# Lqm26/BMCNet-ESR

Measured on AMD Instinct MI355X. Metric: LR-voxel-frames/sec x4 SR train step, NFS-shaped 180x240 (BASELINE configs[1] / [2]), f32, higher is better.
Workload: dtype f32; 1 GPU; BMCNet(scale=4, n_c=128, n_b=5) x4 SR train step, NFS-shaped 180x240 (BASELINE configs[1] / [2]) -> 720x960, bs=4/GPU, arithmetic fp32 (native fp32 MFMA; 3x3 convolutions through Winograd F(4x4,3x3) / F(2x2,3x3) transforms in fp32), SEQL=9 SEQN=2 (8 windows BPTT), event scatter + fwd + MSE + bwd + Adam(amsgrad); global_batch=4, parallelism=dp1, rccl_ranks=1, rccl_initialised_before_headline_run=False

## Files before the change

### bmcnet-esr_amd/csrc/wino4_wgrad.hip

```cpp
#include "bmc_common.h"
#include "dma_ring.h"

namespace {

struct Wgrad4K {
    SrcDev a;
    SrcDev x;
    int B, H, W;
    int TY, SX;
    int nstages, nsplit;
    float* part;
    float* bias_part;
};

typedef float f32x2 __attribute__((ext_vector_type(2)));

__device__ __forceinline__ const float* uni(const float* p) {
    const unsigned long long v = reinterpret_cast<unsigned long long>(p);
    const unsigned lo = __builtin_amdgcn_readfirstlane((unsigned)v), hi = __builtin_amdgcn_readfirstlane((unsigned)(v >> 32));
    return reinterpret_cast<const float*>(((unsigned long long)hi << 32) | lo);
}

constexpr int NPW = 18;
constexpr int TS = 4;
constexpr int CH = 64;
constexpr int PIMG = TS * CH;
constexpr int IMG = NPW * PIMG;
constexpr int SIMG = 2 * IMG;
constexpr int XPC = 23, YPC = 16;
constexpr int RAWX = XPC * 256;
constexpr int RAWF = (XPC + YPC) * 256;
constexpr int NPC = XPC + YPC;
constexpr int PPW = 5;
constexpr int LDSF = 2 * RAWF + 2 * SIMG;
static_assert(LDSF * 4 <= 160 * 1024, "LDS budget");

constexpr int dma_gap(const int j) { return 2 * j; }
constexpr int TR_READ = 0, TR_COMB = 3, TR_OUT = 10;

template <int I, int N>
struct W4gFor {
    template <class F>
    static __device__ __forceinline__ void run(F&& f) {
        f(std::integral_constant<int, I>{});
        W4gFor<I + 1, N>::run(f);
    }
};
template <int N>
struct W4gFor<N, N> {
    template <class F>
    static __device__ __forceinline__ void run(F&&) {}
};

template <int TG, int ROLE>
__device__ __forceinline__ void wgrad4_body(const Wgrad4K& a, float* const lds, const int split, const int chh, const int kh) {
    const int tid = threadIdx.x, lane = tid & 63;
    const int wave = __builtin_amdgcn_readfirstlane(tid >> 6);
    float* const rawb = lds;
    float* const imgb = lds + 2 * RAWF;
    const unsigned lds_raw = lds_addr(rawb);

    const int pg = wave >> 2, cb = (wave >> 1) & 1, kb = wave & 1;
    const int l31 = lane & 31, lh = lane >> 5;
    const int aoff = 3 * pg * PIMG + lh * CH + 32 * cb + l31;
    const int boff = IMG + 3 * pg * PIMG + lh * CH + 32 * kb + l31;
    f32x16 acc[9];
#pragma unroll
    for (int i = 0; i < 9; ++i)
#pragma unroll
        for (int r = 0; r < 16; ++r) acc[i][r] = 0.f;

    unsigned poff[PPW];
    unsigned pof[PPW];
    unsigned pla[PPW];
    unsigned pxm = 0;
    auto piece_of = [&](const int j) { return min(wave + 8 * j, NPC - 1); };
    const bool has_last = wave + 8 * (PPW - 1) < NPC;
    auto slot_of = [&](const int p, int& r, int& c) __attribute__((always_inline)) {
        if (p < XPC) { const int q = 4 * p + (lane >> 4); r = q / 18; c = q - 18 * r; return q < 90; }
        const int q = 4 * (p - XPC) + (lane >> 4); r = q >> 4; c = q & 15;
        return true;
    };
#pragma unroll
    for (int j = 0; j < PPW; ++j) {
        const int p = piece_of(j);
        int r, c;
        const bool real = slot_of(p, r, c);
        poff[j] = real ? (unsigned)(((r * a.W + c) * 128 + (lane & 15) * 4) * 4) : 0u;
        pof[j] = poff[j];
        pla[j] = lds_raw + (unsigned)(p * 1024);
        pxm |= p < XPC ? 1u << j : 0u;
    }
    unsigned zm = 0;
    static_assert(PPW <= 32, "zm is a bit mask");

    const int per_img = a.TY * a.SX;
    const int st0 = (int)((long long)a.nstages * split / a.nsplit), st1 = (int)((long long)a.nstages * (split + 1) / a.nsplit);
    int nb = st0 / per_img, nty, nsx;
    {
        const int r = st0 - nb * per_img;
        nty = r / a.SX; nsx = r - nty * a.SX;
    }
    nb = __builtin_amdgcn_readfirstlane(nb); nty = __builtin_amdgcn_readfirstlane(nty); nsx = __builtin_amdgcn_readfirstlane(nsx);
    const float* xbat = nullptr;
    const float* ybat = nullptr;
    const float* xrow = nullptr;
    const float* yrow = nullptr;
    bool rowborder = false;
    auto row_setup = [&]() __attribute__((always_inline)) {
        xbat = uni(src_batch_ptr(a.x, nb) + kh * CH);
        ybat = uni(src_batch_ptr(a.a, nb) + chh * CH);
        const int y0 = 4 * nty - 1 + TG;
        rowborder = y0 < 0 || y0 + 4 >= a.H;
        xrow = xbat + (long long)y0 * a.W * 128;
        yrow = ybat + (long long)(4 * nty) * a.W * 128;
    };
    row_setup();

    const float* rq_xs = nullptr;
    const float* rq_ys = nullptr;
    unsigned rq_lo = 0;
    auto rq_begin = [&](const int rb) __attribute__((always_inline)) {
        rq_lo = (unsigned)(rb * RAWF * 4);
        const int y0 = 4 * nty - 1 + TG, x0 = 16 * nsx - 1;
        const bool border = rowborder || nsx == 0 || x0 + 17 >= a.W;
        rq_xs = border ? xbat : xrow + x0 * 128;
        rq_ys = border ? ybat : yrow + (x0 + 1) * 128;
        zm = 0;
        if (border) {
            asm volatile("; image border" ::: "memory");
#pragma unroll
            for (int j = 0; j < PPW; ++j) {
                const bool isx = (pxm >> j) & 1;
                int r, c;
                const bool real = slot_of(piece_of(j), r, c);
                const int y = (isx ? y0 : y0 + 1 - TG) + r, x = (isx ? x0 : x0 + 1) + c;
                const bool inside = y >= 0 && y < a.H && x >= 0 && x < a.W;
                const int yc = min(max(y, 0), a.H - 1), xc = min(max(x, 0), a.W - 1);
                pof[j] = real ? (unsigned)(((yc * a.W + xc) * 128 + (lane & 15) * 4) * 4) : 0u;
                zm |= (real && !inside) ? (1u << j) : 0u;
            }
        } else {
#pragma unroll
            for (int j = 0; j < PPW; ++j) pof[j] = poff[j];
        }
        if (!has_last) zm &= ~(1u << (PPW - 1));
        if (++nsx == a.SX) {
            nsx = 0;
            if (++nty == a.TY) { nty = 0; ++nb; }
            row_setup();
        }
    };
    auto rq_piece = [&](const int j) __attribute__((always_inline)) {
        if (j == PPW - 1 && !has_last) return;
        dma16_sgpr<1>(((pxm >> j) & 1) ? rq_xs : rq_ys, pof[j], pla[j] + rq_lo);
    };
    auto patch = [&](const int rb) __attribute__((always_inline)) {
        if (__builtin_amdgcn_ballot_w64(zm != 0) == 0) return;
#pragma unroll
        for (int j = 0; j < PPW; ++j)
            if ((zm >> j) & 1) *reinterpret_cast<f32x4*>(rawb + (pla[j] - lds_raw) / 4 + rb * RAWF + lane * 4) = f32x4{0.f, 0.f, 0.f, 0.f};
    };

    const int pt = 2 * (wave >> 2) + (lane >> 5), cp = lane & 31;
    constexpr int NK = ROLE == 0 ? 3 : 4;
    constexpr int NC = ROLE == 3 ? 4 : 6;
    constexpr int KS = ROLE == 0 ? 2 * 18 * CH : (ROLE == 3 ? 16 * CH : 18 * CH);
    const int tsrc = (ROLE == 0 ? 4 * pt * CH : (ROLE == 3 ? RAWX + 4 * pt * CH : ((1 - TG) * 18 + 4 * pt) * CH)) + 2 * cp;
    const int tdst = (ROLE == 3 ? 0 : IMG + (ROLE == 0 ? (TG == 0 ? 0 : 2) : (TG == 0 ? 1 : 0) + (ROLE == 2 ? 1 : 0)) * 6 * PIMG) + pt * CH + 2 * cp;
    f32x2 td[NC][NK];
    f32x2 tw[3][NC];
    f32x2 bsum = {0.f, 0.f};
    auto ld2 = [](const float* p) __attribute__((always_inline)) { return *reinterpret_cast<const f32x2*>(p); };
    auto st2 = [](float* p, const f32x2 v) __attribute__((always_inline)) { *reinterpret_cast<f32x2*>(p) = v; };
    auto tgap = [&](auto gc, const float* const raw, float* const img) __attribute__((always_inline)) {
        constexpr int G = decltype(gc)::value;
        constexpr int cr = G - TR_READ, cc = G - TR_COMB;
        if constexpr (cr >= 0 && cr < NC) {
#pragma unroll
            for (int k = 0; k < NK; ++k) td[cr][k] = ld2(raw + tsrc + k * KS + cr * CH);
        }
        if constexpr (cc >= 0 && cc < NC) {
            const f32x2* const d = td[cc];
            if constexpr (ROLE == 0) {
                tw[0][cc] = 4.f * d[0] - 5.f * d[1] + d[2];
            } else if constexpr (ROLE < 3) {
                constexpr float al = TG == 0 ? -4.f : -1.f;
                constexpr float ga = (TG == 0 ? 1.f : 2.f) * (ROLE == 2 ? -1.f : 1.f);
                tw[0][cc] = (d[3] + al * d[1]) + ga * (d[2] + al * d[0]);
            } else {
                constexpr float ka = TG == 0 ? 1.f : 4.f, la = TG == 0 ? 1.f : 2.f;
                const f32x2 p = d[0] + ka * d[2], q = d[1] + ka * d[3];
                if (TG == 0) { tw[0][cc] = d[0]; tw[1][cc] = p + la * q; tw[2][cc] = p - la * q; }
                else { tw[0][cc] = p + la * q; tw[1][cc] = p - la * q; tw[2][cc] = d[3]; }
            }
        }
        constexpr int ko = G - TR_OUT;
        if constexpr (ko >= 0 && ko < 6 && (ko & 1) == 0) {
            constexpr int k = ko >> 1;
            if constexpr (ROLE < 3) {
                const f32x2* const w = tw[0];
                float* const dst = img + tdst;
                if (k == 0) {
                    st2(dst, 4.f * w[0] - 5.f * w[2] + w[4]);
                    st2(dst + 5 * PIMG, 4.f * w[1] - 5.f * w[3] + w[5]);
                } else if (k == 1) {
                    const f32x2 ta = w[4] - 4.f * w[2], tb = w[3] - 4.f * w[1];
                    st2(dst + PIMG, ta + tb);
                    st2(dst + 2 * PIMG, ta - tb);
                } else {
                    const f32x2 tc = w[4] - w[2], te = w[3] - w[1];
                    st2(dst + 3 * PIMG, tc + 2.f * te);
                    st2(dst + 4 * PIMG, tc - 2.f * te);
                }
            } else {
                const f32x2* const w = tw[k];
                float* const dst = img + tdst + 6 * k * PIMG;
                const f32x2 s = w[0] + w[2], t = w[1] + w[3], p = w[0] + 4.f * w[2], q = w[1] + 4.f * w[3];
                const f32x2 m1 = s + t;
                st2(dst, w[0]);
                st2(dst + PIMG, m1);
                st2(dst + 2 * PIMG, s - t);
                st2(dst + 3 * PIMG, p + 2.f * q);
                st2(dst + 4 * PIMG, p - 2.f * q);
                st2(dst + 5 * PIMG, w[3]);
                if (TG == 0 && k == 1) bsum += m1;
            }
        }
    };

    auto stage = [&](const int it, auto reqc, auto morec) __attribute__((always_inline)) {
        constexpr bool REQ = decltype(reqc)::value, MORE = decltype(morec)::value;
        const float* const img = imgb + (it & 1) * SIMG;
        const float* const traw = rawb + ((it + 1) & 1) * RAWF;
        float* const timg = imgb + ((it + 1) & 1) * SIMG;
        if (REQ) rq_begin(it & 1);
        float af[3][2], bf[3][2];
        auto frag = [&](const int i) __attribute__((always_inline)) {
            const int u = i / 3, j = i - 3 * u, sl = i % 3;
#pragma unroll
            for (int ks = 0; ks < 2; ++ks) {
                af[sl][ks] = img[aoff + (6 * u + j) * PIMG + 2 * ks * CH];
                bf[sl][ks] = img[boff + (6 * u + j) * PIMG + 2 * ks * CH];
            }
        };
        __builtin_amdgcn_sched_barrier(0);
        frag(0);
        frag(1);
        W4gFor<0, 9>::run([&](auto ic) __attribute__((always_inline)) {
            constexpr int i = decltype(ic)::value;
            __builtin_amdgcn_sched_barrier(0);
            if (i + 2 < 9) frag(i + 2);
            __builtin_amdgcn_sched_barrier(0);
            W4gFor<0, 2>::run([&](auto kc) __attribute__((always_inline)) {
                constexpr int ks = decltype(kc)::value, g = 2 * i + ks;
                acc[i] = __builtin_amdgcn_mfma_f32_32x32x2f32(af[i % 3][ks], bf[i % 3][ks], acc[i], 0, 0, 0);
                if (REQ) {
#pragma unroll
                    for (int j = 0; j < PPW; ++j)
                        if (dma_gap(j) == g) rq_piece(j);
                }
                if (MORE) tgap(std::integral_constant<int, g>{}, traw, timg);
                __builtin_amdgcn_sched_barrier(0);
            });
        });
        dma_wait<0>();
        if (REQ) patch(it & 1);
        ring_publish();
    };

    const int n = st1 - st0;
    if (n <= 0) return;
    rq_begin(0);
#pragma unroll
    for (int j = 0; j < PPW; ++j) rq_piece(j);
    dma_wait<0>();
    patch(0);
    ring_publish();
    if (n > 1) {
        rq_begin(1);
#pragma unroll
        for (int j = 0; j < PPW; ++j) rq_piece(j);
    }
    W4gFor<0, 18>::run([&](auto gc) __attribute__((always_inline)) { tgap(gc, rawb, imgb); });
    dma_wait<0>();
    if (n > 1) patch(1);
    ring_publish();
    using T_ = std::true_type;
    using F_ = std::false_type;
    int it = 0;
    for (; it + 2 < n; ++it) stage(it, T_{}, T_{});
    if (it + 1 < n) stage(it++, F_{}, T_{});
    stage(it, F_{}, F_{});

    {
        float* const P = a.part + ((((long long)split * 8 + (TG * 4 + chh * 2 + kh)) * 8 + wave) * 9) * 1024 + lane * 4;
#pragma unroll
        for (int i = 0; i < 9; ++i)
#pragma unroll
            for (int m = 0; m < 4; ++m)
                stg16(P + (i * 4 + m) * 256, f32x4{acc[i][4 * m], acc[i][4 * m + 1], acc[i][4 * m + 2], acc[i][4 * m + 3]});
    }
    if (TG == 0 && kh == 0 && a.bias_part) {
        if (ROLE == 3) *reinterpret_cast<f32x2*>(lds + pt * CH + 2 * cp) = bsum;
        __syncthreads();
        if (tid < CH) a.bias_part[(long long)split * 128 + 64 * chh + tid] = (lds[tid] + lds[CH + tid]) + (lds[2 * CH + tid] + lds[3 * CH + tid]);
    }
}

template <int TG>
__device__ __forceinline__ void wgrad4_role(const Wgrad4K& a, float* const lds, const int split, const int chh, const int kh) {
    switch (__builtin_amdgcn_readfirstlane(threadIdx.x >> 6) & 3) {
        case 0: wgrad4_body<TG, 0>(a, lds, split, chh, kh); break;
        case 1: wgrad4_body<TG, 1>(a, lds, split, chh, kh); break;
        case 2: wgrad4_body<TG, 2>(a, lds, split, chh, kh); break;
        default: wgrad4_body<TG, 3>(a, lds, split, chh, kh); break;
    }
}

__global__ __launch_bounds__(512, 2) void wino4_wgrad_kernel(const Wgrad4K a) {
    __shared__ __attribute__((aligned(16))) float lds[LDSF];
    int type, split;
    if ((a.nsplit & 7) == 0) {
        const int j = blockIdx.x >> 3;
        type = j & 7; split = (j >> 3) * 8 + (blockIdx.x & 7);
    } else {
        type = blockIdx.x & 7; split = blockIdx.x >> 3;
    }
    const int chh = (type >> 1) & 1, kh = type & 1;
    if (type & 4) wgrad4_role<1>(a, lds, split, chh, kh);
    else wgrad4_role<0>(a, lds, split, chh, kh);
}

constexpr int RED_THREADS = 288, RED_GROUPS = 512;
__global__ __launch_bounds__(RED_THREADS) void wino4_wgrad_reduce_kernel(const float* __restrict__ part, int nsplit, float* __restrict__ dw,
                                                                        int ldw, int k0, int accumulate, const float* __restrict__ bias_part,
                                                                        float* __restrict__ db) {
    constexpr long long SSTRIDE = 36ll * 16384;
    const int t = threadIdx.x;
    if ((int)blockIdx.x == RED_GROUPS) {
        if (t >= 128) return;
        float s = 0.f;
        int i = 0;
        for (; i + 8 <= nsplit; i += 8) {
            float q[8];
#pragma unroll
            for (int k = 0; k < 8; ++k) q[k] = bias_part[(long long)(i + k) * 128 + t];
#pragma unroll
            for (int k = 0; k < 8; ++k) s += q[k];
        }
        for (; i < nsplit; ++i) s += bias_part[(long long)i * 128 + t];
        db[t] = accumulate ? db[t] + s : s;
        return;
    }
    __shared__ f32x4 U[36][8];
    const int c = blockIdx.x >> 5, r = blockIdx.x & 31;
    const int chh = c >> 3, kh = (c >> 2) & 1, cb = (c >> 1) & 1, kb = c & 1;
    const int m = r >> 3, lane0 = 8 * (r & 7);
    {
        const int p = t >> 3, qi = t & 7;
        const int xi = p / 6, nu = p - 6 * xi;
        const int type = (xi / 3) * 4 + chh * 2 + kh, wv = (nu / 3) * 4 + cb * 2 + kb, a9 = 3 * (xi % 3) + nu % 3;
        const float* const ps = part + (((long long)type * 8 + wv) * 9 + a9) * 1024 + m * 256 + (lane0 + qi) * 4;
        f32x4 u = {0.f, 0.f, 0.f, 0.f};
        int s = 0;
        for (; s + 8 <= nsplit; s += 8) {
            f32x4 q[8];
#pragma unroll
            for (int k = 0; k < 8; ++k) q[k] = ldg16(ps + (s + k) * SSTRIDE);
#pragma unroll
            for (int k = 0; k < 8; ++k) u += q[k];
        }
        for (; s < nsplit; ++s) u += ldg16(ps + s * SSTRIDE);
        U[p][qi] = u;
    }
    __syncthreads();
    const float G[6][3] = {{0.25f, 0.f, 0.f}, {-1.f / 6, -1.f / 6, -1.f / 6}, {-1.f / 6, 1.f / 6, -1.f / 6},
                           {1.f / 24, 1.f / 12, 1.f / 6}, {1.f / 24, -1.f / 12, 1.f / 6}, {0.f, 0.f, 1.f}};
    const int e = t / 72, r2 = t - 72 * e, qi = r2 / 9, tap = r2 - 9 * qi, ti = tap / 3, tj = tap - 3 * ti;
    float o = 0.f;
#pragma unroll
    for (int k = 0; k < 8; ++k) {
        float tk = 0.f;
#pragma unroll
        for (int p = k; p < 36; p += 8) {
            const int xi = p / 6, nu = p - 6 * xi;
            float gi = 0.f, gj = 0.f;
#pragma unroll
            for (int q = 0; q < 3; ++q) { gi = q == ti ? G[xi][q] : gi; gj = q == tj ? G[nu][q] : gj; }
            tk += (gi * gj) * U[p][qi][e];
        }
        o += tk;
    }
    const int co = 64 * chh + 32 * cb + 8 * m + 4 * (lane0 >> 5) + e, ci = 64 * kh + 32 * kb + (lane0 & 31) + qi;
    float* const d = dw + ((long long)co * ldw + k0 + ci) * 9 + tap;
    *d = accumulate ? *d + o : o;
}

}

static long long w4g_stages(int B, int H, int W) { return (long long)B * ((H + 3) / 4) * (((W + 3) / 4 + TS - 1) / TS); }

extern "C" int bmc_wgrad_wino4_nsplit(int B, int H, int W) {
    if (B < 1 || H < 1 || W < 1) return 0;
    const long long stages = w4g_stages(B, H, W);
    const int per_type = bmc_num_cus() / 8 > 0 ? bmc_num_cus() / 8 : 1;
    return (int)(stages < per_type ? stages : per_type);
}

extern "C" int bmc_wgrad_wino4(const bmc_src_t* dy, const bmc_src_t* x, int B, int H, int W, int nsplit, float* part,
                               float* bias_part, bmc_stream_t s) {
    BMC_CHECK_ARG(dy && x && part && dy->ptr && x->ptr, "bmc_wgrad_wino4: null argument");
    BMC_CHECK_ARG(dy->nch == 128 && x->nch == 128, "bmc_wgrad_wino4: both operands must be 128-channel windows (got %d, %d)", dy->nch,
                  x->nch);
    BMC_CHECK_ARG(dy->pix_stride == 128 && x->pix_stride == 128, "bmc_wgrad_wino4: both operands must be dense in the channel axis "
                  "(pix_stride 128; got %d, %d)", dy->pix_stride, x->pix_stride);
    BMC_CHECK_ARG(B >= 1 && H >= 1 && W >= 1 && (long long)H * W * 128 < (1ll << 29), "bmc_wgrad_wino4: bad geometry");
    Wgrad4K k;
    k.a = to_dev(*dy); k.x = to_dev(*x);
    k.B = B; k.H = H; k.W = W;
    k.TY = (H + 3) / 4; k.SX = ((W + 3) / 4 + TS - 1) / TS;
    const long long stages = w4g_stages(B, H, W);
    BMC_CHECK_ARG(stages < (1ll << 31), "bmc_wgrad_wino4: too many tiles");
    BMC_CHECK_ARG(nsplit >= 1 && nsplit <= stages, "bmc_wgrad_wino4: nsplit must be in [1, %lld]", stages);
    k.nstages = (int)stages; k.nsplit = nsplit;
    k.part = part; k.bias_part = bias_part;
    hipLaunchKernelGGL(wino4_wgrad_kernel, dim3((unsigned)nsplit * 8), dim3(512), 0, (hipStream_t)s, k);
    BMC_CHECK_LAUNCH("bmc_wgrad_wino4");
    return 0;
}

extern "C" int bmc_wgrad_wino4_reduce(const float* part, int nsplit, float* dw, int ldw, int k0, int accumulate,
                                      const float* bias_part, float* db, bmc_stream_t s) {
    BMC_CHECK_ARG(part && dw && nsplit >= 1, "bmc_wgrad_wino4_reduce: bad arguments");
    BMC_CHECK_ARG(ldw >= 128 && k0 >= 0 && k0 + 128 <= ldw, "bmc_wgrad_wino4_reduce: columns [k0, k0 + 128) must lie inside the %d input "
                  "channels of the weight tensor", ldw);
    BMC_CHECK_ARG((bias_part == nullptr) == (db == nullptr), "bmc_wgrad_wino4_reduce: bias_part and db go together");
    hipLaunchKernelGGL(wino4_wgrad_reduce_kernel, dim3(RED_GROUPS + (bias_part ? 1 : 0)), dim3(RED_THREADS), 0, (hipStream_t)s, part, nsplit, dw, ldw, k0,
                       accumulate, bias_part, db);
    BMC_CHECK_LAUNCH("bmc_wgrad_wino4_reduce");
    return 0;
}
```

Measured before the change: 47.86 LR-voxel-frames/s.

## Move stage barrier inside MFMA loop and prefetch next stage fragments early

The DMA wait, border patch and ring barrier move from the end of each wgrad stage to a fixed MFMA gap (gap 15), after the transform writes. The first two fragment loads for the next stage are issued right after that barrier, and the next request's address state is computed at gap 16 instead of at the start of the stage. Border handling now uses packed precomputed row/column slots and a shared base offset, which makes the per-piece border math cheaper. The aim is to hide barrier and LDS-load latency behind the remaining MFMAs. The cost is a more fragile schedule that rests on static gap ordering, plus an extra publish at the end.

```diff
diff --git a/bmcnet-esr_amd/csrc/wino4_wgrad.hip b/bmcnet-esr_amd/csrc/wino4_wgrad.hip
--- a/bmcnet-esr_amd/csrc/wino4_wgrad.hip
+++ b/bmcnet-esr_amd/csrc/wino4_wgrad.hip
@@ -37,6 +37,10 @@
 
 constexpr int dma_gap(const int j) { return 2 * j; }
 constexpr int TR_READ = 0, TR_COMB = 3, TR_OUT = 10;
+constexpr int BAR_GAP = 15, RQ_GAP = 16;
+static_assert(dma_gap(4) < BAR_GAP, "every piece is issued in front of the stage's wait");
+static_assert(RQ_GAP >= BAR_GAP && RQ_GAP <= 17, "the next request's state is made in place, behind the patch of the one before");
+static_assert(TR_OUT + 4 <= BAR_GAP && BAR_GAP >= 15 && BAR_GAP <= 17, "the barrier follows the transform's writes; fragment registers");
 
 template <int I, int N>
 struct W4gFor {
@@ -74,6 +78,7 @@
     unsigned pof[PPW];
     unsigned pla[PPW];
     unsigned pxm = 0;
+    unsigned prc[2] = {0, 0};
     auto piece_of = [&](const int j) { return min(wave + 8 * j, NPC - 1); };
     const bool has_last = wave + 8 * (PPW - 1) < NPC;
     auto slot_of = [&](const int p, int& r, int& c) __attribute__((always_inline)) {
@@ -90,9 +95,10 @@
         pof[j] = poff[j];
         pla[j] = lds_raw + (unsigned)(p * 1024);
         pxm |= p < XPC ? 1u << j : 0u;
+        prc[j >> 2] |= (real ? (unsigned)(r | c << 3) : 0u) << (8 * (j & 3));
     }
     unsigned zm = 0;
-    static_assert(PPW <= 32, "zm is a bit mask");
+    static_assert(PPW <= 8, "two registers of slots");
 
     const int per_img = a.TY * a.SX;
     const int st0 = (int)((long long)a.nstages * split / a.nsplit), st1 = (int)((long long)a.nstages * (split + 1) / a.nsplit);
@@ -119,9 +125,7 @@
 
     const float* rq_xs = nullptr;
     const float* rq_ys = nullptr;
-    unsigned rq_lo = 0;
-    auto rq_begin = [&](const int rb) __attribute__((always_inline)) {
-        rq_lo = (unsigned)(rb * RAWF * 4);
+    auto rq_next = [&]() __attribute__((always_inline)) {
         const int y0 = 4 * nty - 1 + TG, x0 = 16 * nsx - 1;
         const bool border = rowborder || nsx == 0 || x0 + 17 >= a.W;
         rq_xs = border ? xbat : xrow + x0 * 128;
@@ -129,31 +133,31 @@
         zm = 0;
         if (border) {
             asm volatile("; image border" ::: "memory");
+            const int yy0 = y0 + 1 - TG, yx0 = x0 + 1;
+            const unsigned xbase = (unsigned)((y0 * a.W + x0) * 512), ybase = (unsigned)((yy0 * a.W + yx0) * 512);
 #pragma unroll
             for (int j = 0; j < PPW; ++j) {
                 const bool isx = (pxm >> j) & 1;
-                int r, c;
-                const bool real = slot_of(piece_of(j), r, c);
-                const int y = (isx ? y0 : y0 + 1 - TG) + r, x = (isx ? x0 : x0 + 1) + c;
-                const bool inside = y >= 0 && y < a.H && x >= 0 && x < a.W;
-                const int yc = min(max(y, 0), a.H - 1), xc = min(max(x, 0), a.W - 1);
-                pof[j] = real ? (unsigned)(((yc * a.W + xc) * 128 + (lane & 15) * 4) * 4) : 0u;
-                zm |= (real && !inside) ? (1u << j) : 0u;
+                const unsigned rc = prc[j >> 2] >> (8 * (j & 3));
+                const int y = (isx ? y0 : yy0) + (int)(rc & 7), x = (isx ? x0 : yx0) + (int)((rc >> 3) & 31);
+                const bool inside = (unsigned)y < (unsigned)a.H && (unsigned)x < (unsigned)a.W;
+                pof[j] = inside ? (isx ? xbase : ybase) + poff[j] : 0u;
+                zm |= inside ? 0u : 1u << j;
             }
+            if (!has_last) zm &= ~(1u << (PPW - 1));
         } else {
 #pragma unroll
             for (int j = 0; j < PPW; ++j) pof[j] = poff[j];
         }
-        if (!has_last) zm &= ~(1u << (PPW - 1));
         if (++nsx == a.SX) {
             nsx = 0;
             if (++nty == a.TY) { nty = 0; ++nb; }
             row_setup();
         }
     };
-    auto rq_piece = [&](const int j) __attribute__((always_inline)) {
+    auto rq_piece = [&](const int j, const int rb) __attribute__((always_inline)) {
         if (j == PPW - 1 && !has_last) return;
-        dma16_sgpr<1>(((pxm >> j) & 1) ? rq_xs : rq_ys, pof[j], pla[j] + rq_lo);
+        dma16_sgpr<1>(((pxm >> j) & 1) ? rq_xs : rq_ys, pof[j], pla[j] + (unsigned)(rb * RAWF * 4));
     };
     auto patch = [&](const int rb) __attribute__((always_inline)) {
         if (__builtin_amdgcn_ballot_w64(zm != 0) == 0) return;
@@ -229,28 +233,25 @@
         }
     };
 
+    float af[3][2], bf[3][2];
+    auto frag = [&](const float* const img, const int i) __attribute__((always_inline)) {
+        const int u = i / 3, j = i - 3 * u, sl = i % 3;
+#pragma unroll
+        for (int ks = 0; ks < 2; ++ks) {
+            af[sl][ks] = img[aoff + (6 * u + j) * PIMG + 2 * ks * CH];
+            bf[sl][ks] = img[boff + (6 * u + j) * PIMG + 2 * ks * CH];
+        }
+    };
+    const int n = st1 - st0;
     auto stage = [&](const int it, auto reqc, auto morec) __attribute__((always_inline)) {
         constexpr bool REQ = decltype(reqc)::value, MORE = decltype(morec)::value;
         const float* const img = imgb + (it & 1) * SIMG;
         const float* const traw = rawb + ((it + 1) & 1) * RAWF;
         float* const timg = imgb + ((it + 1) & 1) * SIMG;
-        if (REQ) rq_begin(it & 1);
-        float af[3][2], bf[3][2];
-        auto frag = [&](const int i) __attribute__((always_inline)) {
-            const int u = i / 3, j = i - 3 * u, sl = i % 3;
-#pragma unroll
-            for (int ks = 0; ks < 2; ++ks) {
-                af[sl][ks] = img[aoff + (6 * u + j) * PIMG + 2 * ks * CH];
-                bf[sl][ks] = img[boff + (6 * u + j) * PIMG + 2 * ks * CH];
-            }
-        };
-        __builtin_amdgcn_sched_barrier(0);
-        frag(0);
-        frag(1);
         W4gFor<0, 9>::run([&](auto ic) __attribute__((always_inline)) {
             constexpr int i = decltype(ic)::value;
             __builtin_amdgcn_sched_barrier(0);
-            if (i + 2 < 9) frag(i + 2);
+            if (i + 2 < 9) frag(img, i + 2);
             __builtin_amdgcn_sched_barrier(0);
             W4gFor<0, 2>::run([&](auto kc) __attribute__((always_inline)) {
                 constexpr int ks = decltype(kc)::value, g = 2 * i + ks;
@@ -258,40 +259,50 @@
                 if (REQ) {
 #pragma unroll
                     for (int j = 0; j < PPW; ++j)
-                        if (dma_gap(j) == g) rq_piece(j);
+                        if (dma_gap(j) == g) rq_piece(j, it & 1);
                 }
                 if (MORE) tgap(std::integral_constant<int, g>{}, traw, timg);
+                if (MORE && g == BAR_GAP) {
+                    if (REQ) {
+                        dma_wait<0>();
+                        patch(it & 1);
+                    }
+                    ring_publish();
+                    frag(timg, 0);
+                    frag(timg, 1);
+                }
+                if (REQ && g == RQ_GAP) rq_next();
                 __builtin_amdgcn_sched_barrier(0);
             });
         });
-        dma_wait<0>();
-        if (REQ) patch(it & 1);
-        ring_publish();
-    };
-
-    const int n = st1 - st0;
+    };
+
     if (n <= 0) return;
-    rq_begin(0);
-#pragma unroll
-    for (int j = 0; j < PPW; ++j) rq_piece(j);
+    rq_next();
+#pragma unroll
+    for (int j = 0; j < PPW; ++j) rq_piece(j, 0);
     dma_wait<0>();
     patch(0);
     ring_publish();
     if (n > 1) {
-        rq_begin(1);
-#pragma unroll
-        for (int j = 0; j < PPW; ++j) rq_piece(j);
+        rq_next();
+#pragma unroll
+        for (int j = 0; j < PPW; ++j) rq_piece(j, 1);
     }
     W4gFor<0, 18>::run([&](auto gc) __attribute__((always_inline)) { tgap(gc, rawb, imgb); });
     dma_wait<0>();
     if (n > 1) patch(1);
+    if (n > 2) rq_next();
     ring_publish();
+    frag(imgb, 0);
+    frag(imgb, 1);
     using T_ = std::true_type;
     using F_ = std::false_type;
     int it = 0;
     for (; it + 2 < n; ++it) stage(it, T_{}, T_{});
     if (it + 1 < n) stage(it++, F_{}, T_{});
     stage(it, F_{}, F_{});
+    ring_publish();
 
     {
         float* const P = a.part + ((((long long)split * 8 + (TG * 4 + chh * 2 + kh)) * 8 + wave) * 9) * 1024 + lane * 4;
```

Measured after the change: 48.12 LR-voxel-frames/s, median of 6. No clear change (+0.6%).
